# OpenDriveLab/ThinkTwice

Hardware: AMD Instinct MI355X
Metric: frames/sec forward (4-cam+LiDAR, thinktwice.py cfg) (higher is better)
Workload: dtype bf16x3h; 1 GPU; forward_inference thinktwice.py cfg: 8 frames x (2 sweeps x 4 cams x 448x896 + 65536-pt LiDAR), ResNet50+PAFPN+DepthNet+UNet+LSS splat, LidarNet, fusion, 5-stage decoder; parallelism=replicas x1 (no data-path collective), launch=eager launches, 3 batches in flight on alternating streams, batches_in_flight=3

## Files before the change

### include/thinktwice_hip.h

```cpp
#ifndef THINKTWICE_HIP_H
#define THINKTWICE_HIP_H

#include <stddef.h>
#include <stdint.h>

#ifdef __cplusplus
extern "C" {
#endif

#define TT_F32 0
#define TT_BF16 1
#define TT_F16 2

#define TT_ACT_NONE 0
#define TT_ACT_RELU 1
#define TT_ACT_SIGMOID 2
#define TT_ACT_GELU 3
#define TT_ACT_SOFTPLUS 4
#define TT_ACT_SOFTPLUS_CLAMP 5

const char* tt_last_error(void);
const char* tt_conv_last_kernel(void);
int tt_conv_set_trace(void* stamps_or_null);
int tt_version(void);
// ... 160 lines not shown
                   int x_stride, int out_stride, int act, int dtype, void* stream);
int tt_layernorm_rows(const void* x, const float* gamma, const float* beta, void* out, long long R,
                      int D, int x_stride, int out_stride, float eps, int dtype, void* stream);
int tt_copy_nhwc(const void* in, void* out, int N, int H, int W, int C, int in_cstride, int in_coff,
                 int out_cstride, int out_coff, int rot_flip, int in_dtype, int out_dtype, void* stream);
int tt_broadcast_rows(const void* v, void* out, int N, int HW, int C, int v_stride, int out_cstride,
                      int out_coff, int dtype, void* stream);
int tt_ew(const void* a, const void* b, const void* g, void* out, long long R, int C, int a_stride,
          int a_coff, int b_stride, int b_coff, int g_stride, int g_coff, int o_stride, int o_coff,
          int op, int act, int dtype, void* stream);
int tt_concat_rows(float* out, long long R, int out_stride, int nseg, const float* const* srcs, const int* strides,
                   const int* widths, const int* coffs, const int* divs, const int* mods, void* stream);

int tt_deform_im2col3x3(const void* x, const float* offsets, void* cols, int N, int H, int W, int C,
                        int off_cstride, int pad, int dtype, void* stream);

int tt_look_project_pack(int B, const float* wp, const float* lidar2img, const float* ida_mat,
                         float img_h, float img_w, float* ref_packed, int* query_of_slot,
                         int* count, int* max_len, void* stream);
int tt_look_gather_query(int B, const int* query_of_slot, const float* ref_packed, const float* wp,
                         const float* ctrl_softplus, const float* temporal_embedding,
                         const float* static_embedding, const float* measurement_feat,
                         const float* flattened_feat, const void* const* level_maps,
                         const int* level_hw, int maps_dtype, float* out, int row_stride, void* stream);
int tt_msda_sample(int B, const void* value, int value_dtype, const float* offsets, const float* logits,
                   const float* ref_packed, const int* level_hw, float* out, void* stream);
int tt_msda_sample_strided(int B, const void* value, int value_dtype, int value_cstride, int value_coff,
                           const float* offsets, const float* logits, const float* ref_packed, const int* level_hw,
                           float* out, void* stream);
int tt_sca_reduce(int B, const float* x, const int* max_len, float* out, void* stream);
// ... 399 lines not shown
```

### thinktwice_amd/build.py

```python
import os
import subprocess
import sys
from concurrent.futures import ThreadPoolExecutor

from . import _lib

HERE = os.path.dirname(os.path.abspath(__file__))
CSRC = os.path.join(HERE, "csrc")
OBJ = os.path.join(CSRC, "_obj")
LIB = os.path.join(HERE, "libthinktwice_hip.so")
HIPCC = os.environ.get("HIPCC", "/opt/rocm/bin/hipcc")
FLAGS = ["--offload-arch=gfx950", "-O3", "-std=c++17", "-fPIC", "-munsafe-fp-atomics", "-ffp-contract=off",
         "-Wno-unused-result"]


EXTRA_FLAGS = {"conv_x3_pipe.hip": ["-fno-slp-vectorize"], "conv_x3_up2.hip": ["-fno-slp-vectorize"],
               "conv_x3_patch.hip": ["-fno-slp-vectorize"], "conv_x3_join.hip": ["-fno-slp-vectorize"],
               "conv_x3_stem.hip": ["-fno-slp-vectorize"]}


def _sources():
    return sorted(f for f in os.listdir(CSRC) if f.endswith((".hip", ".cpp")))


def _deps_mtime():
    hdrs = [os.path.join(CSRC, f) for f in os.listdir(CSRC) if f.endswith((".h", ".inc"))]
    hdrs.append(os.path.join(HERE, "..", "include", "thinktwice_hip.h"))
    hdrs.append(os.path.abspath(__file__))
    return max(os.path.getmtime(h) for h in hdrs)


def _compile(src, hdr_mtime, verbose):
    obj = os.path.join(OBJ, src + ".o")
# ... 81 lines not shown
```

### thinktwice_amd/csrc/dcn.hip

```cpp
#include "tt_common.h"

namespace tt {

template <typename T>
__global__ __launch_bounds__(256) void deform_im2col_kernel(const T* __restrict__ x, const float* __restrict__ off,
                                                            T* __restrict__ cols, int N, int H, int W, int C,
                                                            int off_cstride, int pad) {
    constexpr int V = Elem<T>::kVec;
    const int cv = C / V;
    const long long total = (long long)N * H * W * 9 * cv;
    for (long long i = (long long)blockIdx.x * blockDim.x + threadIdx.x; i < total;
         i += (long long)gridDim.x * blockDim.x) {
        const int c = (int)(i % cv);
        long long r = i / cv;
        const int tap = (int)(r % 9);
        const long long pix = r / 9;
        const int xw = (int)(pix % W);
        const int yh = (int)((pix / W) % H);
        const long long n = pix / ((long long)H * W);
        const float dy = off[pix * off_cstride + 2 * tap];
        const float dx = off[pix * off_cstride + 2 * tap + 1];
        const float py = (float)(yh + tap / 3 - pad) + dy;
        const float px = (float)(xw + tap % 3 - pad) + dx;
        float acc[V];
#pragma unroll
        for (int k = 0; k < V; ++k) acc[k] = 0.f;
        if (py > -1.f && py < (float)H && px > -1.f && px < (float)W) {
            const int y0 = (int)floorf(py), x0 = (int)floorf(px);
            const float ly = py - (float)y0, lx = px - (float)x0;
            const float hy = 1.f - ly, hx = 1.f - lx;
            const T* base = x + n * H * W * C + c * V;
            auto add = [&](int yy, int xx, float wgt) {
                if (yy < 0 || yy > H - 1 || xx < 0 || xx > W - 1) return;
                const T* p = base + ((long long)yy * W + xx) * C;
#pragma unroll
                for (int k = 0; k < V; ++k) acc[k] += wgt * Elem<T>::ld(p + k);
            };
            add(y0, x0, hy * hx);
            add(y0, x0 + 1, hy * lx);
            add(y0 + 1, x0, ly * hx);
            add(y0 + 1, x0 + 1, ly * lx);
        }
        T* dst = cols + (pix * 9 + tap) * C + c * V;
#pragma unroll
        for (int k = 0; k < V; ++k) Elem<T>::st(dst + k, acc[k]);
    }
}

}

using namespace tt;

extern "C" int tt_deform_im2col3x3(const void* x, const float* offsets, void* cols, int N, int H, int W, int C,
                                   int off_cstride, int pad, int dtype, void* stream) {
    TT_REQUIRE(x && offsets && cols, "tt_deform_im2col3x3: null");
    const int vec = dtype == TT_F32 ? 4 : 8;
// ... 16 lines not shown
```

### thinktwice_amd/csrc/plan_thunks.inc

```

static int thunk_tt_voxel_pool_fwd(const PlanVal* a, void* stream) { return tt_voxel_pool_fwd((int)a[0].i, (int)a[1].i, (int)a[2].i, (int)a[3].i, (int)a[4].i, (int)a[5].i, (const int32_t*)a[6].p, (const float*)a[7].p, (float*)a[8].p, (int32_t*)a[9].p, stream); }
static int thunk_tt_voxel_pool_fwd_ws(const PlanVal* a, void* stream) { return tt_voxel_pool_fwd_ws((int)a[0].i, (int)a[1].i, (int)a[2].i, (int)a[3].i, (int)a[4].i, (int)a[5].i, (const int32_t*)a[6].p, (const float*)a[7].p, (float*)a[8].p, (int32_t*)a[9].p, (void*)a[10].p, (long long)a[11].i, stream); }
static int thunk_tt_voxel_pool_plan_build(const PlanVal* a, void* stream) { return tt_voxel_pool_plan_build((int)a[0].i, (int)a[1].i, (int)a[2].i, (int)a[3].i, (int)a[4].i, (const int32_t*)a[5].p, (void*)a[6].p, (long long)a[7].i, (void*)a[8].p, (long long)a[9].i, stream); }
static int thunk_tt_voxel_pool_fwd_planned(const PlanVal* a, void* stream) { return tt_voxel_pool_fwd_planned((int)a[0].i, (int)a[1].i, (int)a[2].i, (int)a[3].i, (int)a[4].i, (const void*)a[5].p, (const float*)a[6].p, (float*)a[7].p, (void*)a[8].p, (long long)a[9].i, stream); }
static int thunk_tt_voxel_pool_bwd(const PlanVal* a, void* stream) { return tt_voxel_pool_bwd((int)a[0].i, (int)a[1].i, (int)a[2].i, (int)a[3].i, (int)a[4].i, (const int32_t*)a[5].p, (const float*)a[6].p, (float*)a[7].p, stream); }
static int thunk_tt_frustum_voxel_index(const PlanVal* a, void* stream) { return tt_frustum_voxel_index((int)a[0].i, (int)a[1].i, (int)a[2].i, (int)a[3].i, (int)a[4].i, (const float*)a[5].p, (const float*)a[6].p, (const float*)a[7].p, (const float*)a[8].p, (int32_t*)a[9].p, (float*)a[10].p, stream); }
static int thunk_tt_lift_splat_fwd(const PlanVal* a, void* stream) { return tt_lift_splat_fwd((int)a[0].i, (int)a[1].i, (int)a[2].i, (int)a[3].i, (int)a[4].i, (int)a[5].i, (int)a[6].i, (int)a[7].i, (int)a[8].i, (const void*)a[9].p, (const void*)a[10].p, (int)a[11].i, (const int32_t*)a[12].p, (float*)a[13].p, (int)a[14].i, (int)a[15].i, (int)a[16].i, stream); }
static int thunk_tt_lift_splat_fwd_ws(const PlanVal* a, void* stream) { return tt_lift_splat_fwd_ws((int)a[0].i, (int)a[1].i, (int)a[2].i, (int)a[3].i, (int)a[4].i, (int)a[5].i, (int)a[6].i, (int)a[7].i, (int)a[8].i, (const void*)a[9].p, (const void*)a[10].p, (int)a[11].i, (const int32_t*)a[12].p, (float*)a[13].p, (int)a[14].i, (int)a[15].i, (int)a[16].i, (void*)a[17].p, (long long)a[18].i, stream); }
static int thunk_tt_conv2d_fwd(const PlanVal* a, void* stream) { return tt_conv2d_fwd((const tt_conv_desc*)a[0].p, stream); }
static int thunk_tt_conv2d_fwd_next(const PlanVal* a, void* stream) { return tt_conv2d_fwd_next((const tt_conv_desc*)a[0].p, (const tt_conv_next*)a[1].p, stream); }
static int thunk_tt_seg_feedback_chain(const PlanVal* a, void* stream) { return tt_seg_feedback_chain((const float*)a[0].p, (long long)a[1].i, (int)a[2].i, (int)a[3].i, (const float*)a[4].p, (const float*)a[5].p, (const float*)a[6].p, (int)a[7].i, (const float*)a[8].p, (const void*)a[9].p, (int)a[10].i, (const float*)a[11].p, (const float*)a[12].p, (int)a[13].i, (float*)a[14].p, (int)a[15].i, (int)a[16].i, stream); }
static int thunk_tt_mlp_chain(const PlanVal* a, void* stream) { return tt_mlp_chain((const float*)a[0].p, (long long)a[1].i, (int)a[2].i, (int)a[3].i, (const tt_chain_stage*)a[4].p, (int)a[5].i, stream); }
static int thunk_tt_mlp_chain_wide(const PlanVal* a, void* stream) { return tt_mlp_chain_wide((const float*)a[0].p, (long long)a[1].i, (int)a[2].i, (int)a[3].i, (const tt_chain_stage*)a[4].p, (int)a[5].i, (void*)a[6].p, (long long)a[7].i, stream); }
static int thunk_tt_dec_gru(const PlanVal* a, void* stream) { return tt_dec_gru((int)a[0].i, (const float*)a[1].p, (const float*)a[2].p, (float*)a[3].p, (float*)a[4].p, (const void* const*)a[5].p, (const float* const*)a[6].p, (const float* const*)a[7].p, (const void* const*)a[8].p, (const float* const*)a[9].p, (const void*)a[10].p, (const float*)a[11].p, (const void*)a[12].p, (const float*)a[13].p, stream); }
static int thunk_tt_dec_flatten(const PlanVal* a, void* stream) { return tt_dec_flatten((int)a[0].i, (const float*)a[1].p, (float*)a[2].p, (float*)a[3].p, (float*)a[4].p, (const void* const*)a[5].p, (const float* const*)a[6].p, (const float*)a[7].p, (const float*)a[8].p, stream); }
static int thunk_tt_dec_bev_update(const PlanVal* a, void* stream) { return tt_dec_bev_update((int)a[0].i, (const float*)a[1].p, (const float*)a[2].p, (float*)a[3].p, (long long)a[4].i, (float*)a[5].p, (long long)a[6].i, (float*)a[7].p, (const void*)a[8].p, (const float*)a[9].p, (const void* const*)a[10].p, (const float*)a[11].p, stream); }
static int thunk_tt_nchw_to_nhwc_pad(const PlanVal* a, void* stream) { return tt_nchw_to_nhwc_pad((const float*)a[0].p, (void*)a[1].p, (int)a[2].i, (int)a[3].i, (int)a[4].i, (int)a[5].i, (int)a[6].i, (int)a[7].i, stream); }
static int thunk_tt_nchw_to_nhwc_border(const PlanVal* a, void* stream) { return tt_nchw_to_nhwc_border((const float*)a[0].p, (void*)a[1].p, (int)a[2].i, (int)a[3].i, (int)a[4].i, (int)a[5].i, (int)a[6].i, (int)a[7].i, (int)a[8].i, (int)a[9].i, (int)a[10].i, (int)a[11].i, stream); }
static int thunk_tt_nhwc_to_nchw(const PlanVal* a, void* stream) { return tt_nhwc_to_nchw((const void*)a[0].p, (float*)a[1].p, (int)a[2].i, (int)a[3].i, (int)a[4].i, (int)a[5].i, (int)a[6].i, (int)a[7].i, (int)a[8].i, stream); }
static int thunk_tt_maxpool3x3s2(const PlanVal* a, void* stream) { return tt_maxpool3x3s2((const void*)a[0].p, (void*)a[1].p, (int)a[2].i, (int)a[3].i, (int)a[4].i, (int)a[5].i, (int)a[6].i, stream); }
static int thunk_tt_stem_pool_x3(const PlanVal* a, void* stream) { return tt_stem_pool_x3((const float*)a[0].p, (long long)a[1].i, (long long)a[2].i, (long long)a[3].i, (long long)a[4].i, (long long)a[5].i, (long long)a[6].i, (int)a[7].i, (int)a[8].i, (int)a[9].i, (int)a[10].i, (int)a[11].i, (int)a[12].i, (const void*)a[13].p, (int)a[14].i, (int)a[15].i, (int)a[16].i, (const float*)a[17].p, (const float*)a[18].p, (float*)a[19].p, (long long)a[20].i, (int)a[21].i, stream); }
static int thunk_tt_upsample_nearest_add(const PlanVal* a, void* stream) { return tt_upsample_nearest_add((void*)a[0].p, (const void*)a[1].p, (int)a[2].i, (int)a[3].i, (int)a[4].i, (int)a[5].i, (int)a[6].i, (int)a[7].i, (int)a[8].i, stream); }
static int thunk_tt_bilinear_up2(const PlanVal* a, void* stream) { return tt_bilinear_up2((const void*)a[0].p, (void*)a[1].p, (int)a[2].i, (int)a[3].i, (int)a[4].i, (int)a[5].i, (int)a[6].i, stream); }
static int thunk_tt_bilinear_up2_pair(const PlanVal* a, void* stream) { return tt_bilinear_up2_pair((const float*)a[0].p, (float*)a[1].p, (int)a[2].i, (int)a[3].i, (int)a[4].i, (int)a[5].i, stream); }
static int thunk_tt_spatial_pool(const PlanVal* a, void* stream) { return tt_spatial_pool((const void*)a[0].p, (float*)a[1].p, (int)a[2].i, (int)a[3].i, (int)a[4].i, (int)a[5].i, (int)a[6].i, (int)a[7].i, (int)a[8].i, stream); }
static int thunk_tt_channel_gate(const PlanVal* a, void* stream) { return tt_channel_gate((const void*)a[0].p, (const float*)a[1].p, (const void*)a[2].p, (void*)a[3].p, (int)a[4].i, (int)a[5].i, (int)a[6].i, (int)a[7].i, (int)a[8].i, (int)a[9].i, stream); }
static int thunk_tt_affine_rows(const PlanVal* a, void* stream) { return tt_affine_rows((const void*)a[0].p, (const float*)a[1].p, (const float*)a[2].p, (void*)a[3].p, (long long)a[4].i, (int)a[5].i, (int)a[6].i, (int)a[7].i, (int)a[8].i, (int)a[9].i, stream); }
static int thunk_tt_layernorm_rows(const PlanVal* a, void* stream) { return tt_layernorm_rows((const void*)a[0].p, (const float*)a[1].p, (const float*)a[2].p, (void*)a[3].p, (long long)a[4].i, (int)a[5].i, (int)a[6].i, (int)a[7].i, (float)a[8].d, (int)a[9].i, stream); }
static int thunk_tt_copy_nhwc(const PlanVal* a, void* stream) { return tt_copy_nhwc((const void*)a[0].p, (void*)a[1].p, (int)a[2].i, (int)a[3].i, (int)a[4].i, (int)a[5].i, (int)a[6].i, (int)a[7].i, (int)a[8].i, (int)a[9].i, (int)a[10].i, (int)a[11].i, (int)a[12].i, stream); }
static int thunk_tt_broadcast_rows(const PlanVal* a, void* stream) { return tt_broadcast_rows((const void*)a[0].p, (void*)a[1].p, (int)a[2].i, (int)a[3].i, (int)a[4].i, (int)a[5].i, (int)a[6].i, (int)a[7].i, (int)a[8].i, stream); }
static int thunk_tt_ew(const PlanVal* a, void* stream) { return tt_ew((const void*)a[0].p, (const void*)a[1].p, (const void*)a[2].p, (void*)a[3].p, (long long)a[4].i, (int)a[5].i, (int)a[6].i, (int)a[7].i, (int)a[8].i, (int)a[9].i, (int)a[10].i, (int)a[11].i, (int)a[12].i, (int)a[13].i, (int)a[14].i, (int)a[15].i, (int)a[16].i, stream); }
static int thunk_tt_concat_rows(const PlanVal* a, void* stream) { return tt_concat_rows((float*)a[0].p, (long long)a[1].i, (int)a[2].i, (int)a[3].i, (const float* const*)a[4].p, (const int*)a[5].p, (const int*)a[6].p, (const int*)a[7].p, (const int*)a[8].p, (const int*)a[9].p, stream); }
static int thunk_tt_deform_im2col3x3(const PlanVal* a, void* stream) { return tt_deform_im2col3x3((const void*)a[0].p, (const float*)a[1].p, (void*)a[2].p, (int)a[3].i, (int)a[4].i, (int)a[5].i, (int)a[6].i, (int)a[7].i, (int)a[8].i, (int)a[9].i, stream); }
static int thunk_tt_look_project_pack(const PlanVal* a, void* stream) { return tt_look_project_pack((int)a[0].i, (const float*)a[1].p, (const float*)a[2].p, (const float*)a[3].p, (float)a[4].d, (float)a[5].d, (float*)a[6].p, (int*)a[7].p, (int*)a[8].p, (int*)a[9].p, stream); }
static int thunk_tt_look_gather_query(const PlanVal* a, void* stream) { return tt_look_gather_query((int)a[0].i, (const int*)a[1].p, (const float*)a[2].p, (const float*)a[3].p, (const float*)a[4].p, (const float*)a[5].p, (const float*)a[6].p, (const float*)a[7].p, (const float*)a[8].p, (const void* const*)a[9].p, (const int*)a[10].p, (int)a[11].i, (float*)a[12].p, (int)a[13].i, stream); }
static int thunk_tt_msda_sample(const PlanVal* a, void* stream) { return tt_msda_sample((int)a[0].i, (const void*)a[1].p, (int)a[2].i, (const float*)a[3].p, (const float*)a[4].p, (const float*)a[5].p, (const int*)a[6].p, (float*)a[7].p, stream); }
static int thunk_tt_msda_sample_strided(const PlanVal* a, void* stream) { return tt_msda_sample_strided((int)a[0].i, (const void*)a[1].p, (int)a[2].i, (int)a[3].i, (int)a[4].i, (const float*)a[5].p, (const float*)a[6].p, (const float*)a[7].p, (const int*)a[8].p, (float*)a[9].p, stream); }
static int thunk_tt_sca_reduce(const PlanVal* a, void* stream) { return tt_sca_reduce((int)a[0].i, (const float*)a[1].p, (const int*)a[2].p, (float*)a[3].p, stream); }
static int thunk_tt_look_query_ln(const PlanVal* a, void* stream) { return tt_look_query_ln((int)a[0].i, (const int*)a[1].p, (const float*)a[2].p, (const float*)a[3].p, (const float*)a[4].p, (int)a[5].i, (const float*)a[6].p, (const float*)a[7].p, (const float*)a[8].p, (const float*)a[9].p, (const void* const*)a[10].p, (const int*)a[11].p, (int)a[12].i, (const float*)a[13].p, (const float*)a[14].p, (float)a[15].d, (float*)a[16].p, (int)a[17].i, stream); }
static int thunk_tt_msda_sample_ln(const PlanVal* a, void* stream) { return tt_msda_sample_ln((int)a[0].i, (const void*)a[1].p, (int)a[2].i, (int)a[3].i, (int)a[4].i, (const float*)a[5].p, (const float*)a[6].p, (const float*)a[7].p, (const int*)a[8].p, (const float*)a[9].p, (const float*)a[10].p, (float)a[11].d, (float*)a[12].p, (float*)a[13].p, (const int*)a[14].p, stream); }
static int thunk_tt_msda_sample_proj_ln(const PlanVal* a, void* stream) { return tt_msda_sample_proj_ln((int)a[0].i, (const void* const*)a[1].p, (const int*)a[2].p, (const float*)a[3].p, (const float*)a[4].p, (const float*)a[5].p, (const float*)a[6].p, (const float*)a[7].p, (const float*)a[8].p, (const float*)a[9].p, (const float*)a[10].p, (float)a[11].d, (float*)a[12].p, (float*)a[13].p, (const int*)a[14].p, stream); }
static int thunk_tt_sca_reduce_ln(const PlanVal* a, void* stream) { return tt_sca_reduce_ln((int)a[0].i, (const float*)a[1].p, (const int*)a[2].p, (const float*)a[3].p, (const float*)a[4].p, (float)a[5].d, (float*)a[6].p, stream); }
static int thunk_tt_dec_merge_in(const PlanVal* a, void* stream) { return tt_dec_merge_in((int)a[0].i, (const float*)a[1].p, (const float*)a[2].p, (const float*)a[3].p, (const float*)a[4].p, (const float*)a[5].p, (const float*)a[6].p, (float)a[7].d, (float*)a[8].p, stream); }
static int thunk_tt_lidar_voxelize(const PlanVal* a, void* stream) { return tt_lidar_voxelize((const float*)a[0].p, (int)a[1].i, (int)a[2].i, (int)a[3].i, (const float*)a[4].p, (const float*)a[5].p, (const int*)a[6].p, (int)a[7].i, (int)a[8].i, (void*)a[9].p, (long long)a[10].i, (float*)a[11].p, (int*)a[12].p, (int*)a[13].p, stream); }
static int thunk_tt_lidar_voxelize_capped(const PlanVal* a, void* stream) { return tt_lidar_voxelize_capped((const float*)a[0].p, (int)a[1].i, (int)a[2].i, (int)a[3].i, (const float*)a[4].p, (const float*)a[5].p, (const int*)a[6].p, (int)a[7].i, (int)a[8].i, (int)a[9].i, (void*)a[10].p, (long long)a[11].i, (float*)a[12].p, (int*)a[13].p, (int*)a[14].p, stream); }
static int thunk_tt_sp_volume_build(const PlanVal* a, void* stream) { return tt_sp_volume_build((const int*)a[0].p, (const int*)a[1].p, (long long)a[2].i, (int)a[3].i, (const int*)a[4].p, (int*)a[5].p, stream); }
static int thunk_tt_sp_strided_outputs(const PlanVal* a, void* stream) { return tt_sp_strided_outputs((const int*)a[0].p, (const int*)a[1].p, (long long)a[2].i, (int)a[3].i, (const int*)a[4].p, (const int*)a[5].p, (void*)a[6].p, (long long)a[7].i, (int*)a[8].p, (int*)a[9].p, (int*)a[10].p, (long long)a[11].i, stream); }
static int thunk_tt_sp_rulebook(const PlanVal* a, void* stream) { return tt_sp_rulebook((const int*)a[0].p, (const int*)a[1].p, (long long)a[2].i, (const int*)a[3].p, (const int*)a[4].p, (const int*)a[5].p, (int*)a[6].p, stream); }
// ... 82 lines not shown
    {"tt_nhwc_to_nchw", thunk_tt_nhwc_to_nchw, 9},
    {"tt_maxpool3x3s2", thunk_tt_maxpool3x3s2, 7},
    {"tt_stem_pool_x3", thunk_tt_stem_pool_x3, 22},
    {"tt_upsample_nearest_add", thunk_tt_upsample_nearest_add, 9},
    {"tt_bilinear_up2", thunk_tt_bilinear_up2, 7},
    {"tt_bilinear_up2_pair", thunk_tt_bilinear_up2_pair, 6},
    {"tt_spatial_pool", thunk_tt_spatial_pool, 9},
    {"tt_channel_gate", thunk_tt_channel_gate, 10},
    {"tt_affine_rows", thunk_tt_affine_rows, 10},
    {"tt_layernorm_rows", thunk_tt_layernorm_rows, 10},
    {"tt_copy_nhwc", thunk_tt_copy_nhwc, 13},
    {"tt_broadcast_rows", thunk_tt_broadcast_rows, 9},
    {"tt_ew", thunk_tt_ew, 17},
    {"tt_concat_rows", thunk_tt_concat_rows, 10},
    {"tt_deform_im2col3x3", thunk_tt_deform_im2col3x3, 10},
    {"tt_look_project_pack", thunk_tt_look_project_pack, 10},
    {"tt_look_gather_query", thunk_tt_look_gather_query, 14},
    {"tt_msda_sample", thunk_tt_msda_sample, 8},
    {"tt_msda_sample_strided", thunk_tt_msda_sample_strided, 10},
    {"tt_sca_reduce", thunk_tt_sca_reduce, 4},
    {"tt_look_query_ln", thunk_tt_look_query_ln, 18},
    {"tt_msda_sample_ln", thunk_tt_msda_sample_ln, 15},
    {"tt_msda_sample_proj_ln", thunk_tt_msda_sample_proj_ln, 15},
    {"tt_sca_reduce_ln", thunk_tt_sca_reduce_ln, 7},
    {"tt_dec_merge_in", thunk_tt_dec_merge_in, 9},
    {"tt_lidar_voxelize", thunk_tt_lidar_voxelize, 14},
    {"tt_lidar_voxelize_capped", thunk_tt_lidar_voxelize_capped, 15},
    {"tt_sp_volume_build", thunk_tt_sp_volume_build, 6},
    {"tt_sp_strided_outputs", thunk_tt_sp_strided_outputs, 12},
    {"tt_sp_rulebook", thunk_tt_sp_rulebook, 7},
// ... 64 lines not shown
```

### thinktwice_amd/lss.py

```python
import os

import torch

from . import _lib, camera, layers, ops, weights
from .layers import conv_from_sd, conv_from_weight, deconv2x2_from_sd, linear_from_sd, rows, unrows
from .registry import BACKBONES, NECKS, build_neck


class _ResNet50:

    def __init__(self, sd, p, dtype, device):
        vec = weights.vec_of(dtype)
        self.cin_pad = vec
        self.stem = conv_from_sd(sd, p + ".conv1", dtype, device, bn=p + ".bn1", stride=2, pad=3, act="relu",
                                 cin_pad=vec)
        self.stem_rr, self.stem_rr_x3 = None, None
        if weights.storage_dtype(dtype) != torch.float32:
            w = sd[p + ".conv1.weight"].to(device)
            wr = torch.zeros(w.shape[0], 7, 1, 64, dtype=dtype, device=device)
            wr[:, :, 0, :56] = torch.nn.functional.pad(w.permute(0, 2, 3, 1), (0, 5)).reshape(w.shape[0], 7, 56).to(dtype)
            self.stem_rr = wr.contiguous()
        elif dtype == weights.X3 and os.environ.get("TT_X3_STEM_ROWRUN", "1") == "1":
            w = sd[p + ".conv1.weight"].to(device).float()
            wr = torch.zeros(w.shape[0], 7, 1, 32, dtype=torch.float32, device=device)
# ... 304 lines not shown
        dt, dev = self.dtype, x.device
        cat2 = torch.empty(NI, H0, W0, 384, dtype=dt, device=dev)
        cat3 = torch.empty(NI, H0 // 2, W0 // 2, 512, dtype=dt, device=dev)
        cat4 = torch.empty(NI, H0 // 4, W0 // 4, 512, dtype=dt, device=dev)
        outs = self.img_neck(c, targets=[(cat2, 128), (cat3, 256), (cat4, 256), None])
        return (cat2, cat3, cat4, outs[3][0])

    def _fpn_views(self, bufs):
        cat2, cat3, cat4, e4 = bufs
        return [(cat2, 128, 256), (cat3, 256, 256), (cat4, 256, 256), (e4, 0, 256)]

    def _se_gate(self, name, m):
        fc1, fc2, cr, ce = self.se[name]
        return unrows(ce(cr(fc2(fc1(rows(m))))))

    def _depth_net(self, src, mlp_in, T):
        NI, h, w, _ = src.shape
        dev, dt = src.device, self.dtype
        m24 = torch.zeros(mlp_in.shape[0], 24, dtype=torch.float32, device=dev)
        self.bn22(mlp_in, out=m24, running_updates=T)
        x = self.reduce(src)
        dbg = getattr(self, "_dbg", None)
        if dbg is not None:
            dbg.update(src=src, m24=m24, reduce=x)
        g_ctx = ops.repeat_rows(self._se_gate("context", m24), T)
        g_dep = ops.repeat_rows(self._se_gate("depth", m24), T)
        merge_in = torch.empty(NI, h, w, 384, dtype=dt, device=dev)
        self.context_conv(ops.channel_gate(x, g_ctx), out=merge_in, out_coff=0)
        d = ops.channel_gate(x, g_dep)
        if dbg is not None:
# ... 6 lines not shown
            dbg.update(blocks=d)
        mid = d.shape[-1]
        cat = torch.empty(NI, h, w, 4 * mid, dtype=dt, device=dev)
        pr_cat = x3 and mid % 16 == 0 and ops.pair_ok(NI * h * w, 4 * mid, mid, taps=1)
        for i, br in enumerate(self.aspp):
            br(d, out=cat, out_coff=i * mid, out_pair=pr_cat)
        x5 = self.aspp_gap(rows(ops.spatial_pool(d, 0)))
        self.aspp_gapw.scale = None if layers.BN_TRAIN else self.aspp_out.scale
        shift_n = unrows(self.aspp_gapw(x5)).contiguous()
        d = self.aspp_out(cat, shift_n=shift_n, shift_n_mod=NI, in_pair=pr_cat)
        if dbg is not None:
            dbg.update(aspp_cat=cat, x5=x5, aspp_pre_dropout=d)
        if layers.BN_TRAIN:
            d = ops.dropout(d, 0.5)
        off = self.dcn_off(d, out_dtype=torch.float32)
        cols = ops.deform_im2col3x3(d, off, pad=1)
        dd = torch.empty(NI, h, w, mid, dtype=dt, device=dev)
        cg = mid // self.dcn_groups
        og = self.dcn_w[0].w.shape[0]
        for g, wg in enumerate(self.dcn_w):
            wg(cols, in_coff=g * cg, cin=cg, out=dd.view(NI * h * w, 1, 1, mid), out_coff=g * og)
        depth = self.depth_out(dd, out_dtype=torch.float32)
        return depth, merge_in

    def _seg_net(self, bufs):
        cat2, cat3, cat4, e4 = bufs
        self.up["unet_layer4"](e4, out=cat4, out_coff=0)
        d4 = self.upc["unet_layer4"](cat4)
        self.up["unet_layer3"](d4, out=cat3, out_coff=0)
        d3 = self.upc["unet_layer3"](cat3)
        self.up["unet_layer2"](d3, out=cat2, out_coff=0)
        d2 = self.upc["unet_layer2"](cat2)
        from . import autodiff
        NI, h2, w2, _ = d2.shape
        H, W = 2 * h2, 2 * w2
        fused = autodiff.TAPE is None and not layers.BN_TRAIN and self.dtype == torch.float32
# ... 106 lines not shown
```

### thinktwice_amd/ops.py

```python
import contextlib
import ctypes
import os

import torch

from . import _lib
from ._lib import (TT_BF16, TT_F16, TT_F32, TTError, check, clear_device_faults, cur_stream, device_faults, lib, ptr,
                   raise_on_device_fault, require_cuda)
from . import autodiff


def _active_tape():
    return autodiff.TAPE


def _tape(op, *args):
    tape = _active_tape()
    if tape is not None:
        getattr(tape, op)(*args)


def _st(t):
    return cur_stream(t.device)

# ... 740 lines not shown
                               mods, _st(out)), "tt_concat_rows")
    _tape("concat_rows", o2, pieces, coff)
    return out


def deform_im2col3x3(x, offsets, pad=1):
    N, H, W, C = x.shape
    assert offsets.dtype == torch.float32 and offsets.is_contiguous()
    cols = torch.empty(N * H * W, 1, 9, C, dtype=x.dtype, device=x.device)
    check(lib().tt_deform_im2col3x3(ptr(x), ptr(offsets), ptr(cols), N, H, W, C,
                                    offsets.shape[-1], pad, dtype_code(x), _st(x)), "tt_deform_im2col3x3")
    _tape("deform_im2col3x3", x, offsets, cols, pad)
    return cols


def repeat_rows(t, times):
    assert t.dim() == 2 and t.is_contiguous()
    out = torch.empty(times * t.shape[0], t.shape[1], dtype=t.dtype, device=t.device)
    nb = t.numel() * t.element_size()
    for k in range(times):
        check(lib().tt_copy_bytes(out.data_ptr() + k * nb, ptr(t), nb, _st(t)), "tt_copy_bytes")
    _tape("repeat_rows", t, out, times)
    return out


def look_project_pack(wp, lidar2img, ida_mat, img_hw):
    B = wp.shape[0]
    dev = wp.device
    ref = torch.empty(B, 4, 120, 2, dtype=torch.float32, device=dev)
    qos = torch.empty(B, 4, 120, dtype=torch.int32, device=dev)
# ... 451 lines not shown
```

Measured before the change: 116.3 frames/s.

## Fuse deformable im2col sampling into the grouped 3x3 x3 MFMA conv kernel

Adds a kernel that performs bilinear deformable sampling directly into the MFMA A-operand registers, using precomputed per-tap descriptors in LDS and double-buffered weight tiles. It replaces the separate deform_im2col pass, which wrote a 9x-expanded column buffer, plus the per-group conv launches. This removes that large intermediate buffer's write and read traffic and several launches. In exchange it adds a gather-heavy inner loop that may limit MFMA throughput, and it applies only to f32 storage with 128-channel groups.

```diff
diff --git a/include/thinktwice_hip.h b/include/thinktwice_hip.h
--- a/include/thinktwice_hip.h
+++ b/include/thinktwice_hip.h
@@ -198,6 +198,9 @@
 
 int tt_deform_im2col3x3(const void* x, const float* offsets, void* cols, int N, int H, int W, int C,
                         int off_cstride, int pad, int dtype, void* stream);
+int tt_deform_conv3x3_x3(const float* x, const float* offsets, const void* const* weights_x3, float* out, int N, int H, int W, int C,
+                         int groups, int off_cstride, int x_dtype, int w_cout, int w_kh, int w_kw, int w_cin, int out_cstride,
+                         int out_coff, void* stream);
 
 int tt_look_project_pack(int B, const float* wp, const float* lidar2img, const float* ida_mat,
                          float img_h, float img_w, float* ref_packed, int* query_of_slot,
diff --git a/thinktwice_amd/build.py b/thinktwice_amd/build.py
--- a/thinktwice_amd/build.py
+++ b/thinktwice_amd/build.py
@@ -16,7 +16,7 @@
 
 EXTRA_FLAGS = {"conv_x3_pipe.hip": ["-fno-slp-vectorize"], "conv_x3_up2.hip": ["-fno-slp-vectorize"],
                "conv_x3_patch.hip": ["-fno-slp-vectorize"], "conv_x3_join.hip": ["-fno-slp-vectorize"],
-               "conv_x3_stem.hip": ["-fno-slp-vectorize"]}
+               "conv_x3_stem.hip": ["-fno-slp-vectorize"], "conv_x3_dcn.hip": ["-fno-slp-vectorize"]}
 
 
 def _sources():
diff --git a/thinktwice_amd/csrc/conv_x3_dcn.hip b/thinktwice_amd/csrc/conv_x3_dcn.hip
--- /dev/null
+++ b/thinktwice_amd/csrc/conv_x3_dcn.hip
@@ -0,0 +1,272 @@
+#include "conv_lds_dma.h"
+#include "dcn_sample.h"
+
+namespace tt {
+namespace {
+
+__device__ __forceinline__ void dcn_lds_wait() { asm volatile("s_waitcnt lgkmcnt(0)" ::: "memory"); }
+__device__ __forceinline__ void dcn_pin(u32x4& v) { asm volatile("" : "+v"(v)); }
+
+constexpr int kDcnCg = 128;
+constexpr int kDcnTaps = 9;
+constexpr int kDcnChunks = kDcnCg / 32;
+constexpr int kDcnTiles = kDcnChunks * kDcnTaps;
+constexpr int kDcnTileBytes = kDcnCg * 128;
+constexpr int kDcnWRow = kDcnTaps * kDcnCg;
+
+struct DcnArgs {
+    const float* x;
+    const float* off;
+    const float* w[4];
+    float* out;
+    const void* zero_page;
+    int N, H, W, C, G, off_cstride, M, tiles_m, out_cstride, out_coff;
+};
+
+}
+
+template <int NW>
+__global__ __launch_bounds__(NW * 64, 2) void conv_x3_dcn_kernel(const DcnArgs q) {
+#if defined(__HIP_DEVICE_COMPILE__)
+    constexpr int ROWS = 32 * NW, PPW = 16 / NW;
+    constexpr int RING = 2 * kDcnTileBytes;
+    extern __shared__ __attribute__((aligned(16))) unsigned char smem[];
+    const int tid = threadIdx.x, lane = tid & 63;
+    const int wave = __builtin_amdgcn_readfirstlane(tid >> 6);
+    const int r = lane & 31, half = lane >> 5;
+    const int nblk = q.tiles_m * q.G;
+    if ((int)blockIdx.x >= nblk) return;
+    const int item = xcd_tile(nblk);
+    const int g = item / q.tiles_m, tile = item - g * q.tiles_m;
+    const int Mlim = q.M, H = q.H, W = q.W, C = q.C;
+    const int m0 = tile * ROWS;
+    const unsigned lds_base = (unsigned)(uintptr_t)(__attribute__((address_space(3))) unsigned char*)smem;
+    const unsigned desc_base = lds_base + RING;
+
+    for (int it = tid; it < kDcnTaps * ROWS; it += NW * 64) {
+        const int tap = it / ROWS, row = it - tap * ROWS;
+        const int m = m0 + row < Mlim ? m0 + row : Mlim - 1;
+        const int n = m / (H * W), rem = m - n * (H * W);
+        const int yh = rem / W, xw = rem - yh * W;
+        const float* o = q.off + (long long)m * q.off_cstride + 2 * tap;
+        const DcnTap t = dcn_tap(yh, xw, tap, 1, o[0], o[1], H, W);
+        uint4 d = make_uint4(0u, 0u, 0u, 0u);
+        if (t.inside) {
+            unsigned bits = 16u;
+#pragma unroll
+            for (int c = 0; c < 4; ++c) bits |= dcn_corner_ok(t, c, H, W) ? 1u << c : 0u;
+            d.x = (unsigned)((((n * H + t.y0) * W + t.x0) * C) * 4);
+            d.y = __float_as_uint(t.ly);
+            d.z = __float_as_uint(t.lx);
+            d.w = bits;
+        }
+        *reinterpret_cast<uint4*>(smem + RING + it * 16) = d;
+    }
+    __syncthreads();
+
+    const float* wg = q.w[0];
+    if (g == 1) wg = q.w[1];
+    if (g == 2) wg = q.w[2];
+    if (g == 3) wg = q.w[3];
+    const float* dsrc[PPW];
+#pragma unroll
+    for (int i = 0; i < PPW; ++i) {
+        const int e = (wave + NW * i) * 64 + lane, row = e >> 3, pos = e & 7;
+        dsrc[i] = wg + (long long)row * kDcnWRow + ((pos ^ swz<128>(row)) << 2);
+    }
+    auto issue_tile = [&](int slot, int chunk, int tap) {
+        const unsigned st = lds_base + (unsigned)slot * kDcnTileBytes;
+        const int o = tap * kDcnCg + chunk * 32;
+#pragma unroll
+        for (int i = 0; i < PPW; ++i) dma_piece(dsrc[i] + o, st + (unsigned)(wave + NW * i) * 1024u);
+    };
+
+    const char* const zp = reinterpret_cast<const char*>(q.zero_page);
+    const char* const xg = reinterpret_cast<const char*>(q.x) + (g * kDcnCg + half * 8) * 4;
+    const long long dxB = (long long)C * 4, dyB = (long long)W * C * 4;
+    const unsigned desc_addr = desc_base + (unsigned)(wave * 32 + r) * 16u;
+    float4 ga[4][2][2];
+    auto gather = [&](const u32x4& d, int chunk) {
+        const char* p00 = xg + chunk * 128 + (long long)(int)d.x;
+        const char* pc[4] = {p00, p00 + dxB, p00 + dyB, p00 + dyB + dxB};
+#pragma unroll
+        for (int c = 0; c < 4; ++c) {
+            const char* ptr = (d.w >> c) & 1u ? pc[c] : zp;
+#pragma unroll
+            for (int ks = 0; ks < 2; ++ks) {
+                ga[c][ks][0] = *reinterpret_cast<const float4*>(ptr + ks * 64);
+                ga[c][ks][1] = *reinterpret_cast<const float4*>(ptr + ks * 64 + 16);
+            }
+        }
+    };
+
+    const unsigned fo[2] = {frag_off<128>(r, (unsigned)half), frag_off<128>(r, 4u + (unsigned)half)};
+
+    f32x16 acc[2][1][2];
+    zero_acc(acc[0]);
+    zero_acc(acc[1]);
+
+    issue_tile(0, 0, 0);
+    u32x4 dcur = lds_read(desc_addr);
+    dcn_lds_wait();
+    dcn_pin(dcur);
+    gather(dcur, 0);
+
+    int chunk = 0, tap = 0;
+#pragma unroll 1
+    for (int kt = 0; kt < kDcnTiles; ++kt) {
+        wait_vmcnt<0>();
+        asm volatile("s_barrier" ::: "memory");
+        int nchunk = chunk, ntap = tap + 1;
+        if (ntap == kDcnTaps) {
+            ntap = 0;
+            ++nchunk;
+        }
+        const bool more = kt + 1 < kDcnTiles;
+        const unsigned wb = lds_base + (unsigned)(kt & 1) * kDcnTileBytes;
+        u32x4 dnext = lds_read(desc_addr + (unsigned)(more ? ntap : 0) * (ROWS * 16u));
+
+        float wq[4];
+        dcn_weights(__uint_as_float(dcur.y), __uint_as_float(dcur.z), wq);
+        if (!(dcur.w & 16u)) wq[0] = wq[1] = wq[2] = wq[3] = 0.f;
+        u32x4 ah[2], al[2];
+#pragma unroll
+        for (int ks = 0; ks < 2; ++ks) {
+            float a[8];
+#pragma unroll
+            for (int e = 0; e < 8; ++e) a[e] = 0.f;
+#pragma unroll
+            for (int c = 0; c < 4; ++c) {
+                const float4 v0 = ga[c][ks][0], v1 = ga[c][ks][1];
+                a[0] = dcn_axpy(a[0], wq[c], v0.x); a[1] = dcn_axpy(a[1], wq[c], v0.y);
+                a[2] = dcn_axpy(a[2], wq[c], v0.z); a[3] = dcn_axpy(a[3], wq[c], v0.w);
+                a[4] = dcn_axpy(a[4], wq[c], v1.x); a[5] = dcn_axpy(a[5], wq[c], v1.y);
+                a[6] = dcn_axpy(a[6], wq[c], v1.z); a[7] = dcn_axpy(a[7], wq[c], v1.w);
+            }
+            uint4 hi, lo;
+            split8(a, hi, lo);
+            ah[ks] = __builtin_bit_cast(u32x4, hi);
+            al[ks] = __builtin_bit_cast(u32x4, lo);
+        }
+        dcn_pin(ah[0]); dcn_pin(al[0]); dcn_pin(ah[1]); dcn_pin(al[1]);
+
+        dcn_lds_wait();
+        dcn_pin(dnext);
+        if (more) issue_tile((kt + 1) & 1, nchunk, ntap);
+        else dnext.w = 0u;
+        gather(dnext, more ? nchunk : 0);
+        asm volatile("" ::: "memory");
+        u32x4 bh[4], bl[4];
+#pragma unroll
+        for (int j = 0; j < 4; ++j) {
+            bh[j] = lds_read(wb + (unsigned)j * 4096u + fo[0]);
+            bl[j] = lds_read(wb + (unsigned)j * 4096u + (fo[0] ^ 32u));
+        }
+        dcn_lds_wait();
+#pragma unroll
+        for (int j = 0; j < 4; ++j) {
+            dcn_pin(bh[j]);
+            dcn_pin(bl[j]);
+        }
+
+#pragma unroll
+        for (int ks = 0; ks < 2; ++ks) {
+            const uint4 fh = __builtin_bit_cast(uint4, ah[ks]), fl = __builtin_bit_cast(uint4, al[ks]);
+#pragma unroll
+            for (int j = 0; j < 4; ++j) Mfma<uint16_t>::run(fl, __builtin_bit_cast(uint4, bh[j]), acc[j >> 1][0][j & 1]);
+#pragma unroll
+            for (int j = 0; j < 4; ++j) Mfma<uint16_t>::run(fh, __builtin_bit_cast(uint4, bl[j]), acc[j >> 1][0][j & 1]);
+#pragma unroll
+            for (int j = 0; j < 4; ++j) Mfma<uint16_t>::run(fh, __builtin_bit_cast(uint4, bh[j]), acc[j >> 1][0][j & 1]);
+            if (ks == 0) {
+#pragma unroll
+                for (int j = 0; j < 4; ++j) {
+                    bh[j] = lds_read(wb + (unsigned)j * 4096u + fo[1]);
+                    bl[j] = lds_read(wb + (unsigned)j * 4096u + (fo[1] ^ 32u));
+                }
+                dcn_lds_wait();
+#pragma unroll
+                for (int j = 0; j < 4; ++j) {
+                    dcn_pin(bh[j]);
+                    dcn_pin(bl[j]);
+                }
+            }
+        }
+        dcur = dnext;
+        chunk = nchunk;
+        tap = ntap;
+    }
+
+    __syncthreads();
+    float* sC = reinterpret_cast<float*>(smem) + (tid >> 6) * (32 * (64 + 4));
+    ConvArgs p{};
+    p.out = q.out;
+    p.Cout = C; p.OH = H; p.OW = W; p.M = Mlim;
+    p.out_cstride = q.out_cstride; p.out_coff = q.out_coff;
+    p.shift_n_mod = 1;
+    p.act = TT_ACT_NONE; p.out_dtype = TT_F32;
+    p.out_fast = 1; p.vec_epi = 1; p.res_vec = 1;
+    p.flags = 16;
+    conv_epilogue_vec<float, 4, 1, 2, 32, 64, false>(p, acc[0], sC, lane, tid >> 6, 0, m0, g * kDcnCg, Mlim);
+    conv_epilogue_vec<float, 4, 1, 2, 32, 64, false>(p, acc[1], sC, lane, tid >> 6, 1, m0, g * kDcnCg, Mlim);
+#endif
+}
+
+namespace {
+
+template <int NW>
+int launch_dcn(DcnArgs& q, hipStream_t st) {
+    constexpr size_t loop = 2 * (size_t)kDcnTileBytes + (size_t)kDcnTaps * 32 * NW * 16;
+    constexpr size_t epi = (size_t)NW * 32 * (64 + 4) * 4;
+    constexpr size_t lds = loop > epi ? loop : epi;
+    q.zero_page = zero_page("tt_deform_conv3x3_x3");
+    if (!q.zero_page || lds_opt_in(reinterpret_cast<const void*>(conv_x3_dcn_kernel<NW>), lds, "tt_deform_conv3x3_x3")) return -1;
+    hipLaunchKernelGGL(conv_x3_dcn_kernel<NW>, dim3((unsigned)(q.tiles_m * q.G)), dim3(NW * 64), lds, st, q);
+    return 1;
+}
+
+}
+}
+
+extern "C" int tt_deform_conv3x3_x3(const float* x, const float* offsets, const void* const* weights_x3, float* out, int N, int H, int W,
+                                    int C, int groups, int off_cstride, int x_dtype, int w_cout, int w_kh, int w_kw, int w_cin,
+                                    int out_cstride, int out_coff, void* stream) {
+    using namespace tt;
+    constexpr int NW = 4;
+    TT_REQUIRE(x_dtype == TT_F32, "tt_deform_conv3x3_x3: x_dtype=%d: f32 storage only (the 16-bit and exact-f32 forms keep their two steps)", x_dtype);
+    TT_REQUIRE(x, "tt_deform_conv3x3_x3: x is null");
+    TT_REQUIRE(offsets, "tt_deform_conv3x3_x3: offsets is null");
+    TT_REQUIRE(weights_x3, "tt_deform_conv3x3_x3: weights_x3 is null");
+    TT_REQUIRE(out, "tt_deform_conv3x3_x3: out is null");
+    TT_REQUIRE(N > 0 && H > 0 && W > 0, "tt_deform_conv3x3_x3: N=%d H=%d W=%d must be positive", N, H, W);
+    TT_REQUIRE(groups >= 1 && groups <= 4, "tt_deform_conv3x3_x3: groups=%d must be 1..4", groups);
+    TT_REQUIRE(C > 0 && C % kDcnCg == 0 && C == groups * kDcnCg, "tt_deform_conv3x3_x3: C=%d must be groups * 128 = %d", C, groups * kDcnCg);
+    TT_REQUIRE(w_cout == kDcnCg && w_kh == 1 && w_kw == kDcnTaps && w_cin == kDcnCg,
+               "tt_deform_conv3x3_x3: weights_x3 shape [%d][%d][%d][%d]: a group is [128][1][9][128]", w_cout, w_kh, w_kw, w_cin);
+    for (int g = 0; g < groups; ++g) {
+        TT_REQUIRE(weights_x3[g], "tt_deform_conv3x3_x3: weights_x3[%d] is null", g);
+        TT_REQUIRE(((uintptr_t)weights_x3[g] & 15) == 0, "tt_deform_conv3x3_x3: weights_x3[%d] must be 16-byte aligned", g);
+    }
+    TT_REQUIRE(((uintptr_t)x & 15) == 0, "tt_deform_conv3x3_x3: x must be 16-byte aligned");
+    TT_REQUIRE(off_cstride >= 18, "tt_deform_conv3x3_x3: off_cstride=%d must be at least 18", off_cstride);
+    TT_REQUIRE(((uintptr_t)out & 15) == 0, "tt_deform_conv3x3_x3: out must be 16-byte aligned");
+    TT_REQUIRE(out_cstride > 0 && out_cstride % 4 == 0, "tt_deform_conv3x3_x3: out_cstride=%d must be a positive multiple of 4", out_cstride);
+    TT_REQUIRE(out_coff >= 0 && out_coff % 4 == 0 && out_coff + C <= out_cstride,
+               "tt_deform_conv3x3_x3: out_coff=%d must be a multiple of 4 with out_coff + C <= out_cstride=%d", out_coff, out_cstride);
+    const long long M = (long long)N * H * W;
+    TT_REQUIRE(M * C * 4 < (1ll << 31) && M * off_cstride < (1ll << 31) && M * out_cstride < (1ll << 31),
+               "tt_deform_conv3x3_x3: N=%d H=%d W=%d with C=%d off_cstride=%d out_cstride=%d overflow an int", N, H, W, C, off_cstride,
+               out_cstride);
+
+    DcnArgs q{};
+    q.x = x;
+    q.off = offsets;
+    for (int g = 0; g < groups; ++g) q.w[g] = reinterpret_cast<const float*>(weights_x3[g]);
+    q.N = N; q.H = H; q.W = W; q.C = C; q.G = groups; q.off_cstride = off_cstride; q.M = (int)M;
+    q.tiles_m = div_up(M, 32 * NW);
+    q.out = out; q.out_cstride = out_cstride; q.out_coff = out_coff;
+    const int rc = launch_dcn<NW>(q, (hipStream_t)stream);
+    if (rc < 0) return rc;
+    snprintf(g_conv_kernel, sizeof(g_conv_kernel), "conv_x3_pipe_kernel<dcn, 128>");
+    return check_launch("tt_deform_conv3x3_x3");
+}
diff --git a/thinktwice_amd/csrc/dcn.hip b/thinktwice_amd/csrc/dcn.hip
--- a/thinktwice_amd/csrc/dcn.hip
+++ b/thinktwice_amd/csrc/dcn.hip
@@ -1,4 +1,4 @@
-#include "tt_common.h"
+#include "dcn_sample.h"
 
 namespace tt {
 
@@ -20,26 +20,21 @@
         const long long n = pix / ((long long)H * W);
         const float dy = off[pix * off_cstride + 2 * tap];
         const float dx = off[pix * off_cstride + 2 * tap + 1];
-        const float py = (float)(yh + tap / 3 - pad) + dy;
-        const float px = (float)(xw + tap % 3 - pad) + dx;
+        const DcnTap t = dcn_tap(yh, xw, tap, pad, dy, dx, H, W);
         float acc[V];
 #pragma unroll
         for (int k = 0; k < V; ++k) acc[k] = 0.f;
-        if (py > -1.f && py < (float)H && px > -1.f && px < (float)W) {
-            const int y0 = (int)floorf(py), x0 = (int)floorf(px);
-            const float ly = py - (float)y0, lx = px - (float)x0;
-            const float hy = 1.f - ly, hx = 1.f - lx;
+        if (t.inside) {
+            float wgt[4];
+            dcn_weights(t.ly, t.lx, wgt);
             const T* base = x + n * H * W * C + c * V;
-            auto add = [&](int yy, int xx, float wgt) {
-                if (yy < 0 || yy > H - 1 || xx < 0 || xx > W - 1) return;
-                const T* p = base + ((long long)yy * W + xx) * C;
 #pragma unroll
-                for (int k = 0; k < V; ++k) acc[k] += wgt * Elem<T>::ld(p + k);
-            };
-            add(y0, x0, hy * hx);
-            add(y0, x0 + 1, hy * lx);
-            add(y0 + 1, x0, ly * hx);
-            add(y0 + 1, x0 + 1, ly * lx);
+            for (int q = 0; q < 4; ++q) {
+                if (!dcn_corner_ok(t, q, H, W)) continue;
+                const T* p = base + ((long long)(t.y0 + (q >> 1)) * W + t.x0 + (q & 1)) * C;
+#pragma unroll
+                for (int k = 0; k < V; ++k) acc[k] = dcn_axpy(acc[k], wgt[q], Elem<T>::ld(p + k));
+            }
         }
         T* dst = cols + (pix * 9 + tap) * C + c * V;
 #pragma unroll
diff --git a/thinktwice_amd/csrc/dcn_sample.h b/thinktwice_amd/csrc/dcn_sample.h
--- /dev/null
+++ b/thinktwice_amd/csrc/dcn_sample.h
@@ -0,0 +1,44 @@
+#pragma once
+#include "tt_common.h"
+
+namespace tt {
+
+struct DcnTap {
+    bool inside;
+    int y0, x0;
+    float ly, lx;
+};
+
+__device__ __forceinline__ DcnTap dcn_tap(int yh, int xw, int tap, int pad, float dy, float dx, int H, int W) {
+    const float py = (float)(yh + tap / 3 - pad) + dy;
+    const float px = (float)(xw + tap % 3 - pad) + dx;
+    DcnTap t{false, 0, 0, 0.f, 0.f};
+    if (py > -1.f && py < (float)H && px > -1.f && px < (float)W) {
+        t.inside = true;
+        t.y0 = (int)floorf(py);
+        t.x0 = (int)floorf(px);
+        t.ly = py - (float)t.y0;
+        t.lx = px - (float)t.x0;
+    }
+    return t;
+}
+
+__device__ __forceinline__ void dcn_weights(float ly, float lx, float (&w)[4]) {
+    const float hy = 1.f - ly, hx = 1.f - lx;
+    w[0] = hy * hx;
+    w[1] = hy * lx;
+    w[2] = ly * hx;
+    w[3] = ly * lx;
+}
+
+__device__ __forceinline__ bool dcn_corner_ok(const DcnTap& t, int q, int H, int W) {
+    const int yy = t.y0 + (q >> 1), xx = t.x0 + (q & 1);
+    return !(yy < 0 || yy > H - 1 || xx < 0 || xx > W - 1);
+}
+
+__device__ __forceinline__ float dcn_axpy(float acc, float wgt, float v) {
+#pragma clang fp contract(off)
+    return acc + wgt * v;
+}
+
+}
diff --git a/thinktwice_amd/csrc/plan_thunks.inc b/thinktwice_amd/csrc/plan_thunks.inc
--- a/thinktwice_amd/csrc/plan_thunks.inc
+++ b/thinktwice_amd/csrc/plan_thunks.inc
@@ -32,6 +32,7 @@
 static int thunk_tt_ew(const PlanVal* a, void* stream) { return tt_ew((const void*)a[0].p, (const void*)a[1].p, (const void*)a[2].p, (void*)a[3].p, (long long)a[4].i, (int)a[5].i, (int)a[6].i, (int)a[7].i, (int)a[8].i, (int)a[9].i, (int)a[10].i, (int)a[11].i, (int)a[12].i, (int)a[13].i, (int)a[14].i, (int)a[15].i, (int)a[16].i, stream); }
 static int thunk_tt_concat_rows(const PlanVal* a, void* stream) { return tt_concat_rows((float*)a[0].p, (long long)a[1].i, (int)a[2].i, (int)a[3].i, (const float* const*)a[4].p, (const int*)a[5].p, (const int*)a[6].p, (const int*)a[7].p, (const int*)a[8].p, (const int*)a[9].p, stream); }
 static int thunk_tt_deform_im2col3x3(const PlanVal* a, void* stream) { return tt_deform_im2col3x3((const void*)a[0].p, (const float*)a[1].p, (void*)a[2].p, (int)a[3].i, (int)a[4].i, (int)a[5].i, (int)a[6].i, (int)a[7].i, (int)a[8].i, (int)a[9].i, stream); }
+static int thunk_tt_deform_conv3x3_x3(const PlanVal* a, void* stream) { return tt_deform_conv3x3_x3((const float*)a[0].p, (const float*)a[1].p, (const void* const*)a[2].p, (float*)a[3].p, (int)a[4].i, (int)a[5].i, (int)a[6].i, (int)a[7].i, (int)a[8].i, (int)a[9].i, (int)a[10].i, (int)a[11].i, (int)a[12].i, (int)a[13].i, (int)a[14].i, (int)a[15].i, (int)a[16].i, stream); }
 static int thunk_tt_look_project_pack(const PlanVal* a, void* stream) { return tt_look_project_pack((int)a[0].i, (const float*)a[1].p, (const float*)a[2].p, (const float*)a[3].p, (float)a[4].d, (float)a[5].d, (float*)a[6].p, (int*)a[7].p, (int*)a[8].p, (int*)a[9].p, stream); }
 static int thunk_tt_look_gather_query(const PlanVal* a, void* stream) { return tt_look_gather_query((int)a[0].i, (const int*)a[1].p, (const float*)a[2].p, (const float*)a[3].p, (const float*)a[4].p, (const float*)a[5].p, (const float*)a[6].p, (const float*)a[7].p, (const float*)a[8].p, (const void* const*)a[9].p, (const int*)a[10].p, (int)a[11].i, (float*)a[12].p, (int)a[13].i, stream); }
 static int thunk_tt_msda_sample(const PlanVal* a, void* stream) { return tt_msda_sample((int)a[0].i, (const void*)a[1].p, (int)a[2].i, (const float*)a[3].p, (const float*)a[4].p, (const float*)a[5].p, (const int*)a[6].p, (float*)a[7].p, stream); }
@@ -144,6 +145,7 @@
     {"tt_ew", thunk_tt_ew, 17},
     {"tt_concat_rows", thunk_tt_concat_rows, 10},
     {"tt_deform_im2col3x3", thunk_tt_deform_im2col3x3, 10},
+    {"tt_deform_conv3x3_x3", thunk_tt_deform_conv3x3_x3, 17},
     {"tt_look_project_pack", thunk_tt_look_project_pack, 10},
     {"tt_look_gather_query", thunk_tt_look_gather_query, 14},
     {"tt_msda_sample", thunk_tt_msda_sample, 8},
diff --git a/thinktwice_amd/lss.py b/thinktwice_amd/lss.py
--- a/thinktwice_amd/lss.py
+++ b/thinktwice_amd/lss.py
@@ -342,6 +342,13 @@
         fc1, fc2, cr, ce = self.se[name]
         return unrows(ce(cr(fc2(fc1(rows(m))))))
 
+    def _dcn_fused(self, d, off):
+        from . import autodiff
+        if autodiff.TAPE is not None or layers.BN_TRAIN or self.dtype != torch.float32:
+            return False
+        ws = [wg.w_x3 for wg in self.dcn_w]
+        return all(w is not None for w in ws) and ops.dcn_fused_ok(d, off, ws)
+
     def _depth_net(self, src, mlp_in, T):
         NI, h, w, _ = src.shape
         dev, dt = src.device, self.dtype
@@ -378,12 +385,15 @@
         if layers.BN_TRAIN:
             d = ops.dropout(d, 0.5)
         off = self.dcn_off(d, out_dtype=torch.float32)
-        cols = ops.deform_im2col3x3(d, off, pad=1)
         dd = torch.empty(NI, h, w, mid, dtype=dt, device=dev)
-        cg = mid // self.dcn_groups
-        og = self.dcn_w[0].w.shape[0]
-        for g, wg in enumerate(self.dcn_w):
-            wg(cols, in_coff=g * cg, cin=cg, out=dd.view(NI * h * w, 1, 1, mid), out_coff=g * og)
+        if self._dcn_fused(d, off):
+            ops.deform_conv3x3(d, off, [wg.w_x3 for wg in self.dcn_w], out=dd)
+        else:
+            cols = ops.deform_im2col3x3(d, off, pad=1)
+            cg = mid // self.dcn_groups
+            og = self.dcn_w[0].w.shape[0]
+            for g, wg in enumerate(self.dcn_w):
+                wg(cols, in_coff=g * cg, cin=cg, out=dd.view(NI * h * w, 1, 1, mid), out_coff=g * og)
         depth = self.depth_out(dd, out_dtype=torch.float32)
         return depth, merge_in
 
diff --git a/thinktwice_amd/ops.py b/thinktwice_amd/ops.py
--- a/thinktwice_amd/ops.py
+++ b/thinktwice_amd/ops.py
@@ -778,6 +778,42 @@
     return cols
 
 
+DCN_FUSED = os.environ.get("TT_DCN_FUSED", "1") != "0"
+DCN_FUSED_FLOOR = 4096
+DCN_FUSED_MIN_ROWS = 4097
+
+
+def dcn_fused_ok(x, offsets, weights):
+    if not DCN_FUSED or x.dim() != 4 or offsets.dim() != 4:
+        return False
+    N, H, W, C = x.shape
+    G = len(weights)
+    return (x.dtype == torch.float32 and offsets.dtype == torch.float32 and x.is_contiguous() and offsets.is_contiguous() and
+            tuple(offsets.shape[:3]) == (N, H, W) and offsets.shape[3] >= 18 and 1 <= G <= 4 and C == 128 * G and
+            all(w is not None and w.dtype == torch.float32 and tuple(w.shape) == (128, 1, 9, 128) and w.is_contiguous() for w in weights) and
+            N * H * W >= DCN_FUSED_MIN_ROWS and N * H * W > DCN_FUSED_FLOOR and N * H * W * max(C, offsets.shape[3]) * 4 < 2 ** 31)
+
+
+def deform_conv3x3(x, offsets, weights_x3, out=None, out_coff=0):
+    require_cuda(x, offsets, *weights_x3)
+    N, H, W, C = x.shape
+    G = len(weights_x3)
+    if out is None:
+        out = torch.empty(N, H, W, C, dtype=torch.float32, device=x.device)
+    assert out.dtype == torch.float32 and out.is_contiguous() and out.numel() // out.shape[-1] == N * H * W
+    wp = (ctypes.c_void_p * G)(*[w.data_ptr() for w in weights_x3])
+    w0 = weights_x3[0]
+    with _launch() as rec:
+        check(lib().tt_deform_conv3x3_x3(ptr(x), ptr(offsets), wp, ptr(out), N, H, W, C, G, offsets.shape[-1], dtype_code(x),
+                                         w0.shape[0], w0.shape[1], w0.shape[2], w0.shape[3], out.shape[-1], out_coff, _st(x)),
+              "tt_deform_conv3x3_x3")
+    if rec is not None:
+        M = N * H * W
+        rec.log(2.0 * M * C * 9 * 128, f"M={M} N={C} K=1152 dcn g{G} k3x3s1", kernel=_last_conv_kernel,
+                nbytes=M * (2 * C + 18) * 4 + sum(w.numel() for w in weights_x3) * 4)
+    return out
+
+
 def repeat_rows(t, times):
     assert t.dim() == 2 and t.is_contiguous()
     out = torch.empty(times * t.shape[0], t.shape[1], dtype=t.dtype, device=t.device)
```

Result: no change. 117.3 frames/s, median of 6 (+0.8%).
